# jonathan-laurent/AlphaZero.jl

Hardware: AMD Instinct MI355X
Metric: self-play MCTS sims/sec (Connect-Four, 4096 parallel games per GPU) (higher is better)
Workload: dtype f32

## Files before the change

alphazero.jl_amd/csrc/azhip.hip:

```cpp
#include "engine.h"

static thread_local std::string g_err;
int fail(int code, const char* fmt, ...) {
  char buf[512];
  va_list ap;
  va_start(ap, fmt);
  vsnprintf(buf, sizeof buf, fmt, ap);
  va_end(ap);
  g_err = buf;
  return code;
}
extern "C" const char* az_last_error(void) { return g_err.c_str(); }
extern "C" int az_abi_version(void) { return AZ_ABI_VERSION; }
extern "C" int az_abi_struct_size(int32_t which) {
  switch (which) {
    case AZ_STRUCT_ENGINE_CFG: return (int)sizeof(az_engine_cfg);
    case AZ_STRUCT_MOVE_REC: return (int)sizeof(az_move_rec);
    case AZ_STRUCT_GAME_REC: return (int)sizeof(az_game_rec);
    case AZ_STRUCT_TRACE_BUF: return (int)sizeof(az_trace_buf);
    case AZ_STRUCT_SELFPLAY_STATS: return (int)sizeof(az_selfplay_stats);
    case AZ_STRUCT_SAMPLE: return (int)sizeof(az_sample);
    case AZ_STRUCT_DATASET_INFO: return (int)sizeof(az_dataset_info);
    case AZ_STRUCT_LEARNING_STATUS: return (int)sizeof(az_learning_status_t);
    case AZ_STRUCT_TRAIN_CFG: return (int)sizeof(az_train_cfg);
// ... 48 lines not shown
  c->num_iters_per_turn = 600;
  c->temperature_len = 3;
  c->temperature_xs[0] = 0; c->temperature_xs[1] = 20; c->temperature_xs[2] = 30;
  c->temperature_ys[0] = 1.0; c->temperature_ys[1] = 1.0; c->temperature_ys[2] = 0.3;
  c->num_workers = 128; c->batch_size = 64; c->reset_every = 2; c->fill_batches = 1;
  c->flip_probability = 0.0; c->seed = 1;
  c->num_blocks = 5; c->num_filters = 64; c->num_policy_head_filters = 32; c->num_value_head_filters = 32;
  return AZ_OK;
}

static size_t net_nparams(const GameInfo& gi, const az_engine_cfg& c) {
  size_t P = gi.P, F = c.num_filters, npf = c.num_policy_head_filters, nvf = c.num_value_head_filters;
  size_t s = 9 * (size_t)gi.C * F + 5 * F;
  s += (size_t)c.num_blocks * 2 * (9 * F * F + 5 * F);
  s += F * npf + 5 * npf + (size_t)gi.A * P * npf + gi.A;
  s += F * nvf + 5 * nvf + F * P * nvf + F + F + 1;
  return s;
}

static void drop_wave_graphs(az_engine* e);
extern "C" int az_engine_destroy(az_engine* e) {
  if (!e) return AZ_OK;
  (void)hipSetDevice(e->device);
  if (e->ngroups == 1 && e->fr_s[0] && e->gs[0] == e->fr_s[0]) { for (int i = 0; i < 4; ++i) (void)hipStreamSynchronize(e->fr_s[i]); e->gs[0] = e->gt[0] = e->stream; }
  for (int g = 0; g < e->ngroups; ++g) if (e->gs[g] && e->gs[g] != e->stream) {
    (void)hipStreamSynchronize(e->gt[g]); (void)hipStreamSynchronize(e->gs[g]);
    (void)hipStreamDestroy(e->gt[g]); (void)hipStreamDestroy(e->gs[g]);
    (void)hipEventDestroy(e->ev_tree[g]); (void)hipEventDestroy(e->ev_net[g]);
  }
  if (e->stream) (void)hipStreamSynchronize(e->stream);
  split_register(e, 0);
  if (e->h_xflag) (void)hipHostFree(e->h_xflag);
  if (e->h_nleaf) (void)hipHostFree(e->h_nleaf);
  if (e->h_needy) (void)hipHostFree(e->h_needy);
  if (e->h_fr_words) (void)hipHostFree(e->h_fr_words);
  if (e->h_busy) (void)hipHostFree(e->h_busy);
  for (int i = 0; i < 4; ++i) { if (e->fr_s[i]) { (void)hipStreamSynchronize(e->fr_s[i]); (void)hipStreamDestroy(e->fr_s[i]); } if (e->fr_ev[i]) (void)hipEventDestroy(e->fr_ev[i]); }
  if (e->d_done) (void)hipFree(e->d_done);
  if (e->d_done_off) (void)hipFree(e->d_done_off);
  if (e->h_env) (void)hipHostFree(e->h_env);
  if (e->h_n) (void)hipHostFree(e->h_n);
  if (e->h_pv) (void)hipHostFree(e->h_pv);
  drop_wave_graphs(e);
  for (auto& r : e->prof_pool) { if (r.a) (void)hipEventDestroy(r.a); if (r.b) (void)hipEventDestroy(r.b); }
  for (void* q : e->net_allocs) (void)hipFree(q);
  for (void* q : e->allocs) (void)hipFree(q);
  if (e->d_phase) (void)hipFree(e->d_phase);
  for (size_t i = 0; i < e->vm_handles.size(); ++i) { (void)hipMemUnmap(e->vm_at[i], e->vm_chunk); (void)hipMemRelease(e->vm_handles[i]); }
  if (e->vm_base) (void)hipMemAddressFree(e->vm_base, e->vm_bytes);
  if (e->vmk_base) (void)hipMemAddressFree(e->vmk_base, e->vmk_bytes);
  if (e->stream) (void)hipStreamDestroy(e->stream);
  delete e;
  return AZ_OK;
}

__global__ void k_fill_u32(uint32_t* p, uint32_t val, int n) {
  int i = blockIdx.x * blockDim.x + threadIdx.x;
  if (i < n) p[i] = val;
}
__global__ void k_iota(int* p, int n) {
// ... 72 lines not shown
  if (c->temperature_len < 1 || c->temperature_len > AZ_SCHED_MAX) return fail(AZ_ERR_BAD_ARG, "temperature schedule needs 1..%d breakpoints", AZ_SCHED_MAX);
  if (c->reset_every < 0) return fail(AZ_ERR_BAD_ARG, "reset_every must be >= 0");
  if (c->lock_step != 0 && c->lock_step != 1) return fail(AZ_ERR_BAD_ARG, "lock_step must be 0 (free-running self-play) or 1");
  if (!(c->prior_temperature >= 0.0)) return fail(AZ_ERR_BAD_ARG, "prior_temperature must be >= 0");
  if (c->oracle == AZ_ORACLE_RESNET) {
    if (c->num_filters != 64 && c->num_filters != 128) return fail(AZ_ERR_BAD_ARG, "num_filters = %d: this build instantiates the 64- and 128-filter towers", c->num_filters);
    int hf = c->num_policy_head_filters + c->num_value_head_filters;
    if (c->num_policy_head_filters < 1 || c->num_value_head_filters < 1 || hf > c->num_filters) return fail(AZ_ERR_BAD_ARG, "head filters %d/%d unsupported (policy + value must be <= num_filters)", c->num_policy_head_filters, c->num_value_head_filters);
    if (c->num_blocks < 0 || c->num_blocks > 64) return fail(AZ_ERR_BAD_ARG, "num_blocks out of range");
    if (c->net_bf16 != 0 && c->net_bf16 != 1) return fail(AZ_ERR_BAD_ARG, "net_bf16 must be 0 or 1");
  }
  int ndev = 0;
  HIPCHK(hipGetDeviceCount(&ndev));
  if (c->device < 0 || c->device >= ndev) return fail(AZ_ERR_BAD_ARG, "device %d not available (%d visible)", c->device, ndev);
  HIPCHK(hipSetDevice(c->device));
  az_engine* e = new (std::nothrow) az_engine();
  if (!e) return fail(AZ_ERR_HIP, "out of host memory");
  e->cfg = *c; e->gi = gi; e->device = c->device; e->stream = nullptr; e->ngroups = 0; e->alloc_bytes = 0;
  e->vm_base = nullptr; e->vm_bytes = 0; e->vm_chunk = 0; e->vm_rows = 0; e->vm_chunk_nodes = 0; e->d_slot_cap = nullptr; e->vm_budget = 0; e->vm_mapped = 0;
  e->vmk_base = nullptr; e->vmk_bytes = 0; e->vmk_piece = 0; e->tree_sort = 0; e->d_perm = nullptr; e->d_perm_prev = nullptr;
  e->next_exec = 1.0;
  e->h_env = nullptr; e->h_n = nullptr; e->h_pv = nullptr; e->h_nleaf = nullptr; e->d_nleaf = nullptr; e->h_needy = nullptr; e->d_needy = nullptr;
  e->d_ec = nullptr; e->ec_mask = 0; e->ec_seq = 0; e->d_ec_claim = nullptr; e->d_Phit = nullptr; e->d_Vhit = nullptr;
  e->fr_on = false; e->fr_k = 0; e->fr_kbg = 0; e->fr_round_waves = 0; for (int i = 0; i < 4; ++i) { e->fr_s[i] = nullptr; e->fr_ev[i] = nullptr; } e->d_fr = nullptr; e->d_done = nullptr; e->d_done_off = nullptr; e->done_cap = 0;
  e->h_fr_words = nullptr; e->d_fr_words = nullptr; e->h_busy = nullptr; e->d_busy = nullptr; e->explore_k = 0; e->fr_prev_done = 0; e->fr_since_round = 0; e->fr_given_up = 0; e->fr_prev_recs = 0;
  e->h_xflag = nullptr; e->d_xflag = nullptr; e->split_off = false; e->split_registered = 0; e->xch_launches = 0;
  { const char* fa = getenv("AZHIP_XCH_FAIL_AT"); e->xch_fail_at = fa ? atoll(fa) : 0; }
  e->net_loaded = false; e->running = false; e->prof_on = false; { const char* ug = getenv("AZHIP_GRAPH"); e->use_graphs = ug ? atoi(ug) : 0; }
  e->d_phase = nullptr; e->phase_cap = 0; e->phase_n = 0; e->host_moves = true; e->last_tower[0] = 0; memset(e->tower_hist, 0, sizeof e->tower_hist); e->prof_mask = 0; e->prof_used = 0;
  memset(&e->prof, 0, sizeof e->prof);
  memset(&e->stats, 0, sizeof e->stats);
  int st = [&]() -> int {
    {
      int ncu = 0;
      HIPCHK(hipDeviceGetAttribute(&ncu, hipDeviceAttributeMultiprocessorCount, c->device));
      std::vector<uint32_t> mask((size_t)(ncu + 31) / 32, 0u);
      for (int i = 0; i < ncu; ++i) mask[(size_t)i / 32] |= 1u << (i % 32);
      if (getenv("AZHIP_POOLED_QUEUE") || ncu <= 0 || hipExtStreamCreateWithCUMask(&e->stream, (uint32_t)mask.size(), mask.data()) != hipSuccess) {
        (void)hipGetLastError();
        e->stream = nullptr;
        HIPCHK(hipStreamCreate(&e->stream));
      }
    }
    const int G = c->num_workers;
    DView& v = e->v;
    memset(&v, 0, sizeof v);
    v.G = G;
// ... 158 lines not shown
      gv.G = Gh; gv.slot0 = (int)o;
      gv.sr += o; gv.game_id += o; gv.move_idx += o;
      gv.worker_sim_id += o; gv.eta += o * gi.APAD;
      gv.ht += o * hs; gv.nodes += o * v.node_stride; gv.path += o * v.max_depth;
      if (gv.slot_cap) gv.slot_cap += o;
      gv.leaf_env += o; gv.eval_slots += o; gv.bg_list += o; gv.bg_cnt += 2 * g;
      if (gv.ec) { gv.ec_claim += 2 * o; gv.Phit += o * gi.APAD; gv.Vhit += o; }
      gv.xerr = e->d_xerr + g; gv.skipped = e->d_skipped + 2 * g;
      if (e->tree_sort) {
        gv.perm = e->d_perm + o;
        hipLaunchKernelGGL(k_iota, dim3((Gh + 255) / 256), dim3(256), 0, e->stream, e->d_perm + o, Gh);
      }
      gv.needy_host = e->d_needy + g;
      gv.nleaf_host = e->d_ec ? e->d_nleaf + g : nullptr;
      gv.n_eval += 2 * g; gv.keys += o * v.key_stride; gv.Pout += o * gi.APAD; gv.Vout += o; gv.trace += o * v.max_moves; gv.grec += o; gv.finished += o;
      e->gv[g] = gv;
      if (ng == 1) {
        e->gs[g] = e->gt[g] = e->stream;
        int lo = 0, hi = 0;
        HIPCHK(hipDeviceGetStreamPriorityRange(&lo, &hi));
        HIPCHK(hipStreamCreateWithPriority(&e->fr_s[0], hipStreamNonBlocking, hi));
        HIPCHK(hipStreamCreateWithPriority(&e->fr_s[1], hipStreamNonBlocking, hi));
        HIPCHK(hipStreamCreateWithPriority(&e->fr_s[2], hipStreamNonBlocking, hi));
        HIPCHK(hipStreamCreateWithPriority(&e->fr_s[3], hipStreamNonBlocking, hi));
        for (int i = 0; i < 4; ++i) HIPCHK(hipEventCreateWithFlags(&e->fr_ev[i], hipEventDisableTiming));
      } else {
        int lo = 0, hi = 0;
        HIPCHK(hipDeviceGetStreamPriorityRange(&lo, &hi));
        HIPCHK(hipStreamCreateWithPriority(&e->gs[g], hipStreamNonBlocking, hi));
        HIPCHK(hipStreamCreateWithPriority(&e->gt[g], hipStreamNonBlocking, lo));
        HIPCHK(hipEventCreateWithFlags(&e->ev_tree[g], hipEventDisableTiming));
        HIPCHK(hipEventCreateWithFlags(&e->ev_net[g], hipEventDisableTiming));
      }
      AZCHK(dalloc(e, &e->g_hfeat[g], (size_t)Gh * gi.P * std::max(64, c->num_filters), false));
      e->ngroups = g + 1;
    }
    DParams& p = e->p;
    memset(&p, 0, sizeof p);
    p.gamma = c->gamma; p.cpuct = c->cpuct; p.eps = c->dirichlet_noise_eps; p.alpha = c->dirichlet_noise_alpha;
    p.prior_temp = c->prior_temperature; p.nsims = c->num_iters_per_turn; p.temp_len = c->temperature_len;
    for (int i = 0; i < AZ_SCHED_MAX; ++i) { p.temp_xs[i] = c->temperature_xs[i]; p.temp_ys[i] = c->temperature_ys[i]; }
    p.seed = c->seed; p.oracle = c->oracle; p.reset_every = c->reset_every; p.retire = 0;
    p.flip_p = c->flip_probability;
    if (e->vm_rows) {
      size_t fr = 0, tot = 0;
      HIPCHK(hipMemGetInfo(&fr, &tot));
      const size_t margin = std::max<size_t>(tot / 8, (size_t)4 << 30);
      const char* gb = getenv("AZHIP_POOL_GB");
// ... 455 lines not shown
  if (side) { s2 = e->fr_s[1]; HIPCHK(hipEventRecord(e->fr_ev[0], st)); ++e->bg_seq; e->bg_signal = bg_stop_on && e->fr_kbg > 0; }
  if (e->cfg.oracle == AZ_ORACLE_RESNET) {
    AZCHK(net_wave(e, g, split, e->group_active[g]));
  } else {
    LAUNCH_ON(e, st, AZ_K_SYNTH, G, (k_synth_oracle<Gm>), (G + 255) / 256, 256, 0, v, e->p, sim_idx, par);
  }
  if (e->fr_on) {
    FRArgs fa;
    fa.st = e->d_fr; fa.done = e->d_done; fa.done_off = e->d_done_off;
    fa.recs = e->d_phase ? e->d_phase : e->d_stage; fa.recs_cap = e->d_phase ? (long long)e->phase_cap : (long long)e->v.G * e->v.max_moves;
    fa.done_cap = e->done_cap; fa.total_games = e->total_games; fa.first_game_id = (uint32_t)e->first_game_id; fa.group = g; fa.host_words = e->d_fr_words;
    static const int bg_prio = getenv("AZHIP_BG_PRIO") ? atoi(getenv("AZHIP_BG_PRIO")) : 0;
    hipStream_t s3 = side ? e->fr_s[2] : s2;
    if (side) { HIPCHK(hipStreamWaitEvent(s2, e->fr_ev[0], 0)); HIPCHK(hipStreamWaitEvent(s3, e->fr_ev[0], 0)); }
    { DView mv = v; mv.low_prio = bg_prio ? 0 : 1; LAUNCH_ON(e, s3, AZ_K_MOVE, G, (k_move_fr<Gm>), (G + 255) / 256, 256, 0, mv, e->p, fa); }
    if (e->fr_kbg > 0) {
      AZCHK(ec_next_launch(e, &e->gv[g]));
      DView bv = e->gv[g];
      bv.run_k = e->fr_kbg; bv.low_prio = bg_prio ? 0 : 1;
      if (side && e->bg_signal) { bv.bg_stop = e->d_bg_stop; bv.bg_seq = e->bg_seq; }
      LAUNCH_ON(e, s2, AZ_K_EXPAND, G, (k_tree<Gm>), gb, 256, 0, bv, e->p, 0, 1, par ^ 1);
    }
    if (side) {
      HIPCHK(hipEventRecord(e->fr_ev[1], s2)); HIPCHK(hipStreamWaitEvent(st, e->fr_ev[1], 0));
      HIPCHK(hipEventRecord(e->fr_ev[2], s3)); HIPCHK(hipStreamWaitEvent(st, e->fr_ev[2], 0));
    }
    else if (split && e->cfg.oracle == AZ_ORACLE_RESNET) HIPCHK(hipStreamWaitEvent(st, e->ev_net[g], 0));
  }
  return AZ_OK;
}
template <class Gm> static int recover_split(az_engine* e) {
  AZCHK(sync_all(e));
  *e->h_xflag = 0;
  int xerr[AZ_MAX_GROUPS + 1], skipped[2 * (AZ_MAX_GROUPS + 1)];
  HIPCHK(hipMemcpy(xerr, e->d_xerr, sizeof xerr, hipMemcpyDeviceToHost));
  HIPCHK(hipMemcpy(skipped, e->d_skipped, sizeof skipped, hipMemcpyDeviceToHost));
  HIPCHK(hipMemsetAsync(e->d_xerr, 0, sizeof xerr, e->stream));
  HIPCHK(hipMemsetAsync(e->d_skipped, 0, sizeof skipped, e->stream));
  HIPCHK(hipStreamSynchronize(e->stream));
  bool any = false;
  for (int g = 0; g < e->ngroups; ++g) any = any || xerr[g] == DERR_EXCHANGE;
  if (!any) return AZ_OK;
  e->split_off = true;
  e->stats.tower_fallbacks++;
  for (int g = 0; g < e->ngroups; ++g) {
    e->wave_par[g] ^= (skipped[2 * g] & 1);
    if (skipped[2 * g + 1]) e->pending[g] = true;
  }
// ... 589 lines not shown

extern "C" int az_selfplay_aborted(az_engine* e, int32_t* game_ids, int32_t cap, int32_t* n) {
  ENGINE(e);
  if (!n || (cap > 0 && !game_ids)) return fail(AZ_ERR_BAD_ARG, "NULL");
  *n = (int32_t)e->aborted_ids.size();
  if (*n > cap) return cap == 0 ? AZ_OK : fail(AZ_ERR_CAPACITY, "%d aborted games, room for %d", *n, cap);
  for (int i = 0; i < *n; ++i) game_ids[i] = e->aborted_ids[i];
  return AZ_OK;
}

extern "C" int az_selfplay_end(az_engine* e) {
  ENGINE(e);
  e->p.retire = 0;
  split_register(e, 0);
  if (!e->running) return AZ_OK;
  AZCHK(reset_wave_state(e));
  hipLaunchKernelGGL(k_slot_records, dim3((e->v.G + 255) / 256), dim3(256), 0, e->stream, e->v, (int)SR_CLEAR_ACTIVE);
  HIPCHK(hipStreamSynchronize(e->stream));
  e->running = false;
  e->active_slots = 0;
  e->fr_on = false;
  for (int g = 0; g < e->ngroups; ++g) { e->gv[g].run_k = 0; e->gv[g].fr = 0; e->gv[g].fr_active = nullptr; }
  if (e->ngroups == 1 && e->gs[0] != e->stream) {
    HIPCHK(hipStreamSynchronize(e->gs[0])); for (int i = 1; i < 4; ++i) HIPCHK(hipStreamSynchronize(e->fr_s[i]));
    e->gs[0] = e->gt[0] = e->stream;
  }
  return AZ_OK;
}

extern "C" int az_selfplay_run(az_engine* e, int32_t num_games, int32_t first_game_id, az_trace_buf* out,
                               az_progress_cb cb, void* user, az_selfplay_stats* stats) {
  ENGINE(e);
  if (num_games < 1 || !out) return fail(AZ_ERR_BAD_ARG, "num_games must be >= 1 and out non-NULL");
  if (out->games_cap < num_games) return fail(AZ_ERR_CAPACITY, "games_cap %lld < num_games %d", (long long)out->games_cap, num_games);
  e->host_moves = out->moves != nullptr;
  const int bst = az_selfplay_begin(e, num_games, first_game_id);
  if (bst != AZ_OK) { e->host_moves = true; return bst; }
  int reported = 0;
  int st = AZ_OK;
  while (e->games_done < num_games) {
    st = az_selfplay_step(e, e->fr_on ? e->fr_round_waves : e->p.nsims);
    if (st != AZ_OK) break;
    if (cb) for (; reported < e->games_done; ++reported) cb(user);
  }
  if (st == AZ_OK && stats) st = az_selfplay_get_stats(e, stats);
  std::string keep = g_err;
  const int cst = az_selfplay_collect(e, out);
// ... 257 lines not shown
```

alphazero.jl_amd/csrc/engine.h:

```cpp
#pragma once
#include <hip/hip_runtime.h>

#include <algorithm>
#include <chrono>
#include <cmath>
#include <cstdarg>
#include <cstdio>
#include <cstring>
#include <new>
#include <string>
#include <map>
#include <mutex>
#include <vector>
#include <unordered_set>

#include "../../include/az_numerics.h"
#include "../../include/azhip.h"
#include "games.h"
#include "resnet.h"
#include "resnet16.h"
#include "resnet16b.h"
#include "tree.h"

int fail(int code, const char* fmt, ...);
// ... 71 lines not shown
  int ntm;
  long long tower_hist[4];
  char last_tower[96];
  int heads_pick;
  int tower_pick;
  int num_cu;
  int nn_cap;
  float* d_hfeat; float* d_X; float* d_A; float* d_P; float* d_V; float* d_Pinv;
  GEnv* d_tmp_env; int* d_iota; int* d_ntmp;
  GEnv* h_env; int* h_n; float* h_pv;
  int* d_slots; uint32_t* d_gids; GEnv* d_roots; uint32_t* d_moves; double* d_eta; int* d_offsets;
  az_move_rec* d_stage; unsigned long long* d_keys; int* d_actions; unsigned long long* d_next; signed char* d_term; float* d_reward;
  char* d_nodebuf;
  int* d_visits;
  int io_cap;
  bool running;
  int total_games, next_game, first_game_id, games_done, wave_in_move, active_slots;
  std::map<int, hipGraphExec_t> wave_graphs; int use_graphs;
  bool pending[AZ_MAX_GROUPS];
  int wave_par[AZ_MAX_GROUPS];
  int group_active[AZ_MAX_GROUPS];
  bool fr_on;
  int fr_k, fr_kbg, fr_round_waves;
  hipStream_t fr_s[4]; hipEvent_t fr_ev[4];
  FRState* d_fr; az_game_rec* d_done; long long* d_done_off; int done_cap;
  int* h_busy; int* d_busy;
  int explore_k;
  int* d_bg_stop; int bg_seq; bool bg_signal;
  int* h_fr_words; int* d_fr_words;
  int fr_prev_done, fr_since_round, fr_given_up; long long fr_prev_recs;
  std::vector<az_game_rec> h_done; std::vector<long long> h_done_off;
  std::vector<az_game_rec> q_games;
  std::vector<az_move_rec> q_moves;
  az_move_rec* d_phase; int64_t phase_cap, phase_n; bool host_moves;
  std::vector<az_game_rec> ph_games;
  std::vector<int64_t> ph_off;
  az_selfplay_stats stats;
  std::chrono::steady_clock::time_point t_begin;
  bool prof_on;
  int prof_mask;
  std::vector<ProfRec> prof_pool;
  size_t prof_used;
  az_prof prof;
  double next_exec;
  std::vector<int> h_finished;
  std::vector<az_game_rec> h_grec;
};

template <class T> inline int dalloc(az_engine* e, T** p, size_t n, bool zero = true) {
  void* q = nullptr;
  size_t bytes = std::max<size_t>(n * sizeof(T), 16);
  hipError_t r = hipMalloc(&q, bytes);
  if (r != hipSuccess) return fail(AZ_ERR_HIP, "hipMalloc(%zu bytes) failed: %s", bytes, hipGetErrorString(r));
  e->allocs.push_back(q);
  e->alloc_bytes += bytes;
  if (zero) HIPCHK(hipMemsetAsync(q, 0, bytes, e->stream));
  *p = (T*)q;
  return AZ_OK;
}

inline int sync_groups(az_engine* e) {
  for (int g = 0; g < e->ngroups; ++g) if (e->gs[g] != e->stream) {
    HIPCHK(hipStreamSynchronize(e->gt[g]));
    HIPCHK(hipStreamSynchronize(e->gs[g]));
  }
  if (e->fr_on && e->fr_s[1]) for (int i = 1; i < 4; ++i) HIPCHK(hipStreamSynchronize(e->fr_s[i]));
  return AZ_OK;
}
inline int sync_all(az_engine* e) {
  AZCHK(sync_groups(e));
  HIPCHK(hipStreamSynchronize(e->stream));
  return AZ_OK;
}
inline int prof_flush(az_engine* e) {
  if (!e->prof_used) return AZ_OK;
  AZCHK(sync_all(e));
  for (size_t i = 0; i < e->prof_used; ++i) {
    float ms = 0.f;
    HIPCHK(hipEventElapsedTime(&ms, e->prof_pool[i].a, e->prof_pool[i].b));
    e->prof.ms[e->prof_pool[i].cls] += ms;
  }
  e->prof_used = 0;
  return AZ_OK;
}
inline int prof_begin(az_engine* e, hipStream_t st, int cls, int64_t units) {
  if (!e->prof_on || (e->prof_mask && !((e->prof_mask >> cls) & 1))) return AZ_OK;
  if (e->prof_used == e->prof_pool.size()) AZCHK(prof_flush(e));
  ProfRec& r = e->prof_pool[e->prof_used];
  r.cls = cls;
// ... 64 lines not shown
```

alphazero.jl_amd/csrc/net_impl.h:

```cpp
#pragma once
#include "engine.h"

template <class Gm, int F, bool PLANES_ONLY = false> static int set_kernel_attrs_f() {
  HIPCHK(hipFuncSetAttribute(reinterpret_cast<const void*>(&k_tower16<Gm, F, false>), hipFuncAttributeMaxDynamicSharedMemorySize, T16<Gm, F>::BYTES));
  HIPCHK(hipFuncSetAttribute(reinterpret_cast<const void*>(&k_tower16<Gm, F, true>), hipFuncAttributeMaxDynamicSharedMemorySize, T16<Gm, F>::BYTES));
  if constexpr (NTM<Gm> > 0) {
    HIPCHK(hipFuncSetAttribute(reinterpret_cast<const void*>(&k_tower16<Gm, F, false, NTM<Gm>>), hipFuncAttributeMaxDynamicSharedMemorySize, T16<Gm, F, NTM<Gm>>::BYTES));
    HIPCHK(hipFuncSetAttribute(reinterpret_cast<const void*>(&k_tower16<Gm, F, true, NTM<Gm>>), hipFuncAttributeMaxDynamicSharedMemorySize, T16<Gm, F, NTM<Gm>>::BYTES));
  }
  if constexpr (F == 64) {
    HIPCHK(hipFuncSetAttribute(reinterpret_cast<const void*>(&k_tower16x2<Gm, F, false>), hipFuncAttributeMaxDynamicSharedMemorySize, T16P<Gm, F>::BYTES));
    HIPCHK(hipFuncSetAttribute(reinterpret_cast<const void*>(&k_tower16x2<Gm, F, true>), hipFuncAttributeMaxDynamicSharedMemorySize, T16P<Gm, F>::BYTES));
    HIPCHK(hipFuncSetAttribute(reinterpret_cast<const void*>(&k_tower16x2<Gm, F, false, 10, 9>), hipFuncAttributeMaxDynamicSharedMemorySize, T16P<Gm, F, 10, 9>::BYTES));
    HIPCHK(hipFuncSetAttribute(reinterpret_cast<const void*>(&k_tower16x2<Gm, F, true, 10, 9>), hipFuncAttributeMaxDynamicSharedMemorySize, T16P<Gm, F, 10, 9>::BYTES));
    HIPCHK(hipFuncSetAttribute(reinterpret_cast<const void*>(&k_tower16x2m<Gm, F, false>), hipFuncAttributeMaxDynamicSharedMemorySize, T16P<Gm, F>::BYTES));
    HIPCHK(hipFuncSetAttribute(reinterpret_cast<const void*>(&k_tower16x2c<Gm, F, false>), hipFuncAttributeMaxDynamicSharedMemorySize, T16P<Gm, F>::BYTES));
    HIPCHK(hipFuncSetAttribute(reinterpret_cast<const void*>(&k_tower16x2c<Gm, F, true>), hipFuncAttributeMaxDynamicSharedMemorySize, T16P<Gm, F>::BYTES));
  }
  HIPCHK(hipFuncSetAttribute(reinterpret_cast<const void*>(&k_tower16b<Gm, F, false, 11>), hipFuncAttributeMaxDynamicSharedMemorySize, T16B<Gm, F, 11>::BYTES));
  HIPCHK(hipFuncSetAttribute(reinterpret_cast<const void*>(&k_tower16b<Gm, F, true, 11>), hipFuncAttributeMaxDynamicSharedMemorySize, T16B<Gm, F, 11>::BYTES));
  HIPCHK(hipFuncSetAttribute(reinterpret_cast<const void*>(&k_tower16b<Gm, F, false, NTS<Gm>>), hipFuncAttributeMaxDynamicSharedMemorySize, T16B<Gm, F, NTS<Gm>>::BYTES));
  HIPCHK(hipFuncSetAttribute(reinterpret_cast<const void*>(&k_tower16b<Gm, F, true, NTS<Gm>>), hipFuncAttributeMaxDynamicSharedMemorySize, T16B<Gm, F, NTS<Gm>>::BYTES));
  if constexpr (F == 128) {
    HIPCHK(hipFuncSetAttribute(reinterpret_cast<const void*>(&k_tower16b<Gm, F, false, 22>), hipFuncAttributeMaxDynamicSharedMemorySize, T16B<Gm, F, 22>::BYTES));
// ... 263 lines not shown
        e->next_exec = (first * tower_exec_frac<Gm, F>(e, 21) + (seen - first) * tower_exec_frac<Gm, F>(e, 19)) / (double)seen;
        LAUNCH_ON(e, sn, AZ_K_TOWER, N, (k_tower16x2m<Gm, F, false>), cu + (N - first + T19::TB - 1) / T19::TB, THR21, LDS21, e->net16, v.leaf_env, eslots, nev, N, (const float*)nullptr, e->g_hfeat[g], cu);
        snprintf(e->last_tower, sizeof e->last_tower, "k_tower16x2m<%s,%d>", Gm::ID == 0 ? "ConnectFour" : Gm::ID == 1 ? "TicTacToe" : "Mancala", F);
      } else if (rounds_on && e->tower_pick == 0 && N > first && seen > first && seen + 16 <= first + cu * T19::TB) {
        LAUNCH_ON(e, sn, AZ_K_TOWER, first, (k_tower16x2<Gm, F, false>), cu, THR21, LDS21, e->net16, v.leaf_env, eslots, nev, N, (const float*)nullptr, e->g_hfeat[g], 0);
        e->next_exec = tower_exec_frac<Gm, F>(e, 19);
        LAUNCH_ON(e, sn, AZ_K_TOWER, N - first, (k_tower16x2<Gm, F, false, 10, 9>), (N - first + T19::TB - 1) / T19::TB, (T19::THREADS), (T19::BYTES), e->net16, v.leaf_env, eslots, nev, N, (const float*)nullptr, e->g_hfeat[g], first);
      } else {
        LAUNCH_ON(e, sn, AZ_K_TOWER, N, (k_tower16x2<Gm, F, false>), (N + TB21 - 1) / TB21, THR21, LDS21, e->net16, v.leaf_env, eslots, nev, N, (const float*)nullptr, e->g_hfeat[g], 0);
      }
    }
  } else if (tw == 7) {
    if constexpr (NTM<Gm> > 0) {
      using TM = T16<Gm, F, NTM<Gm>>;
      LAUNCH_ON(e, sn, AZ_K_TOWER, N, (k_tower16<Gm, F, false, NTM<Gm>>), (N + TM::TB - 1) / TM::TB, THR16, (TM::BYTES), e->net16, v.leaf_env, eslots, nev, N, (const float*)nullptr, e->g_hfeat[g]);
    }
  } else if (tw == 3)
    LAUNCH_ON(e, sn, AZ_K_TOWER, N, (k_tower16<Gm, F, false, NTS<Gm>>), (N + TB3 - 1) / TB3, THR16, LDS3, e->net16, v.leaf_env, eslots, nev, N, (const float*)nullptr, e->g_hfeat[g]);
  else if (tw == 16)
    LAUNCH_ON(e, sn, AZ_K_TOWER, N, (k_tower16<Gm, F, false>), (N + TB16 - 1) / TB16, THR16, LDS16, e->net16, v.leaf_env, eslots, nev, N, (const float*)nullptr, e->g_hfeat[g]);
  else
    LAUNCH_ON(e, sn, AZ_K_TOWER, N, (k_tower<Gm, F, false>), (N + TB - 1) / TB, TowerCfg<F>::THREADS, TowerLds<F>::BYTES, e->net, v.leaf_env, eslots, nev, N, (const float*)nullptr, e->g_hfeat[g]);
  const bool fr = e->fr_on && split;
  if (e->bg_signal) {
    HIPCHK(hipEventRecord(e->fr_ev[3], sn));
    HIPCHK(hipStreamWaitEvent(e->fr_s[3], e->fr_ev[3], 0));
    hipLaunchKernelGGL(k_set_word, dim3(1), dim3(1), 0, e->fr_s[3], e->d_bg_stop, e->bg_seq);
  }
  if (split && !fr) { HIPCHK(hipEventRecord(e->ev_net[g], sn)); HIPCHK(hipStreamWaitEvent(st, e->ev_net[g], 0)); }
  AZCHK((launch_heads<Gm, F>(e, fr ? sn : st, e->g_hfeat[g], v.leaf_env, eslots, nev, N, (const float*)nullptr, v.Pout, v.Vout, (float*)nullptr, L)));
  if (fr) HIPCHK(hipEventRecord(e->ev_net[g], sn));
  return AZ_OK;
}
template <class Gm> static int wave_net(az_engine* e, int g, bool split, int nmax) {
  return e->cfg.num_filters == 128 ? wave_net_f<Gm, 128>(e, g, split, nmax) : wave_net_f<Gm, 64>(e, g, split, nmax);
}

#define AZ_NET_GAME_TU(Gm, sfx)                                                                                              \
  int net_set_kernel_attrs_##sfx(az_engine* e) { return set_kernel_attrs<Gm>(e); }                                                      \
  int net_launch_##sfx(az_engine* e, hipStream_t st, bool from_planes, float* hfeat, const GEnv* envs, const int* eslots,    \
                       const int* n_ptr, int n_max, const float* X, const float* Amask, float* Pout, float* Vout, float* Pinv, \
                       int pstride) {                                                                                        \
    return from_planes ? launch_net<Gm, true>(e, st, hfeat, envs, eslots, n_ptr, n_max, X, Amask, Pout, Vout, Pinv, pstride)  \
                       : launch_net<Gm, false>(e, st, hfeat, envs, eslots, n_ptr, n_max, X, Amask, Pout, Vout, Pinv, pstride); \
  }                                                                                                                          \
  int net_wave_##sfx(az_engine* e, int g, bool split, int nmax) { return wave_net<Gm>(e, g, split, nmax); }                  \
  int net_geometry_##sfx(int which, uint16_t* out, int64_t cap, int* rows, int* products) {                                  \
    return which == 0 ? geometry_out<typename T16<Gm, 64, 11>::Geo>(out, cap, rows, products)                                \
         : which == 1 ? geometry_out<typename T16<Gm, 64, NTS<Gm>>::Geo>(out, cap, rows, products)                                 \
         : which == 2 ? geometry_out<typename T16P<Gm, 64>::Geo>(out, cap, rows, products)                                   \
                      : geometry_out<typename T16B<Gm, 128, 22>::Geo>(out, cap, rows, products);                             \
  }
```

alphazero.jl_amd/csrc/resnet.h:

```cpp
#pragma once
#include <hip/hip_runtime.h>
#include <stdint.h>
#include "../../include/az_numerics.h"
#include "games.h"

typedef float f32x16 __attribute__((ext_vector_type(16)));
typedef float f32x4v __attribute__((ext_vector_type(4)));

template <int I, int N, class Fn> __device__ __forceinline__ void static_for_impl(Fn& f) {
  if constexpr (I < N) { f(std::integral_constant<int, I>{}); static_for_impl<I + 1, N>(f); }
}
template <int N, class Fn> __device__ __forceinline__ void static_for(Fn f) { static_for_impl<0, N>(f); }

struct NetDev {
  int nblocks, F, npf, nvf, HF;
  const float* stem_w;
  const float* stem_ss;
  const float4* conv_w;
  const float* conv_ss;
  const float4* head_w;
  const float* head_ss;
  const float* pol_w;
  const float* pol_b;
  const float* val_w;
  const float* val_b;
  const float* val2_w;
  float val2_b;
  unsigned long long* dbg;
  const float2* hd_w;
  int hd_ok;
  const float4* hd16_w;
  int hd16_ok;
};

static constexpr int TOWER_ROWS = 128;

template <int F> struct TowerLds {
  static constexpr int STRIDE = F + 4;
  static constexpr int BUF = (TOWER_ROWS + 1) * STRIDE;
  static constexpr int BYTES = 2 * BUF * 4;
};

template <int F>
__device__ __forceinline__ void load_b_tap(const float4* __restrict__ wt, float4 (&b)[F / 8]) {
#pragma unroll
  for (int jq = 0; jq < F / 8; ++jq) b[jq] = wt[(size_t)jq * 64];
}
template <int F>
__device__ __forceinline__ void mfma_tap(const float4 (&af)[2], const float* __restrict__ arow0,
                                         const float* __restrict__ arow1, const float4 (&b)[F / 8], f32x16 (&acc)[2]) {
#pragma unroll
  for (int c0 = 0; c0 < F / 8; c0 += 8) {
    float4 a0[8], a1[8];
#pragma unroll
    for (int jq = 0; jq < 8; ++jq) {
      if (c0 == 0 && jq == 0) { a0[0] = af[0]; a1[0] = af[1]; }
// ... 249 lines not shown
  av = av + net.val2_b;
  Vout[e] = az_tanhf(av);
}
template <class Gm, int F>
__device__ __forceinline__ void heads_finish(const NetDev& net, const GEnv* __restrict__ leaf_env, const int* __restrict__ eval_slots,
                                             const float* __restrict__ Amask, float* __restrict__ Pout, float* __restrict__ Vout,
                                             float* __restrict__ Pinv, int pstride, int e, const float* __restrict__ logit, const float* __restrict__ vh) {
  heads_finish_policy<Gm>(leaf_env, eval_slots, Amask, Pout, Pinv, pstride, e, logit);
  heads_finish_value<F>(net, Vout, e, vh);
}

template <class Gm> constexpr int HEADS_LP = (Gm::A + 15) / 16 * 16;
template <class Gm> constexpr int HEADS_NPT = (Gm::A + 31) / 32;
template <class Gm, int F>
__global__ void __launch_bounds__(4 * (F + HEADS_LP<Gm>))
k_heads(NetDev net, const GEnv* __restrict__ leaf_env, const int* __restrict__ eval_slots,
        const int* __restrict__ n_eval_ptr, int n_fixed, const float* __restrict__ Amask,
        const float* __restrict__ hfeat, float* __restrict__ Pout, float* __restrict__ Vout,
        float* __restrict__ Pinv, int pstride) {
  constexpr int P = Gm::P, A = Gm::A, HB = 4, PER = F + HEADS_LP<Gm>;
  static_assert(F + A <= PER, "thread map");
  __shared__ float s_logit[HB][HEADS_LP<Gm>];
  __shared__ float s_vh[HB][F];
  const int n = n_eval_ptr ? *n_eval_ptr : n_fixed;
  const int board0 = blockIdx.x * HB;
  if (board0 >= n) return;
  const int b = threadIdx.x / PER, o = threadIdx.x % PER;
  const int e = board0 + b;
  const int HF = net.HF;
  if (e < n && o < F + A) {
    const float* hf = hfeat + (size_t)e * P * HF;
    float acc = 0.0f;
    if (o < F) {
      const int nvf = net.nvf;
      const float* w = net.val_w + o;
      for (int q = 0; q < P; ++q) {
        const float* h = hf + q * HF + net.npf;
        for (int f = 0; f < nvf; ++f) acc = az_fmaf(h[f], w[(size_t)(q * nvf + f) * F], acc);
      }
      acc = acc + net.val_b[o];
      s_vh[b][o] = acc > 0.0f ? acc : 0.0f;
    } else {
      const int a = o - F, npf = net.npf;
      const float* w = net.pol_w + a;
      for (int q = 0; q < P; ++q) {
        const float* h = hf + q * HF;
// ... 67 lines not shown
  for (int r = 0; r < 16; ++r) {
    const int row = (r & 3) + 8 * (r >> 2) + 4 * h;
    if (is_pol) { if (pt * 32 + col < A) s_logit[row * LP + pt * 32 + col] = acc[r] + net.pol_b[pt * 32 + col]; }
    else {
      const int o = wave * 32 + col;
      const float v = acc[r] + net.val_b[o];
      s_vh[row * SV + o] = v > 0.0f ? v : 0.0f;
    }
  }
  }
  __syncthreads();
  const int b = threadIdx.x;
  if (b < 32 && board0 + b < n) heads_finish<Gm, F>(net, leaf_env, eval_slots, Amask, Pout, Vout, Pinv, pstride, board0 + b, s_logit + b * LP, s_vh + b * SV);
}
template <class Gm, int F>
__global__ void __launch_bounds__(64 * (F / 32 + HEADS_NPT<Gm>))
k_heads_mfma(NetDev net, const GEnv* __restrict__ leaf_env, const int* __restrict__ eval_slots,
             const int* __restrict__ n_eval_ptr, int n_fixed, const float* __restrict__ Amask,
             const float* __restrict__ hfeat, float* __restrict__ Pout, float* __restrict__ Vout,
             float* __restrict__ Pinv, int pstride) {
  __builtin_amdgcn_s_setprio(3);
  __shared__ float s_vh[32 * (F + 1)];
  __shared__ float s_logit[32 * HEADS_LP<Gm>];
  const int n = n_eval_ptr ? *n_eval_ptr : n_fixed;
  const int board0 = blockIdx.x * 32;
  if (board0 >= n) return;
  heads_mfma_tile<Gm, F>(net, leaf_env, eval_slots, n, Amask, hfeat, Pout, Vout, Pinv, pstride, board0, s_vh, s_logit);
}

#ifndef HEADS16_DEPTH
#define HEADS16_DEPTH 8
#endif
#ifndef HEADS16_WDEPTH
#define HEADS16_WDEPTH 16
#endif
template <class Gm> constexpr int HEADS16_NPT = (Gm::A + 15) / 16;
template <class Gm, int F, bool SPLIT> struct H16 {
  static constexpr int P = Gm::P, NVT = F / 16, NPT = HEADS16_NPT<Gm>;
  static constexpr int WAVES = SPLIT ? (NVT > NPT ? NVT : NPT) : NVT + NPT, THREADS = 64 * WAVES;
  static constexpr int NB = 2 * P, RS = 20, SV = F + 1, LP = HEADS_LP<Gm>;
  static constexpr bool STAGE = SPLIT && 16 * P * 32 * 4 <= 96 * 1024;
  static constexpr int A_FLOATS = STAGE ? NB * 256 : 0, PATCH_FLOATS = STAGE ? 0 : WAVES * 3 * 16 * RS;
  static constexpr int BYTES = (A_FLOATS + PATCH_FLOATS + 16 * SV + 16 * LP) * 4;
};
template <class Gm, int F, bool SPLIT> struct H16Threads { static constexpr int V = H16<Gm, F, SPLIT>::THREADS; };
template <class Gm, int F, bool SPLIT>
__global__ void __launch_bounds__((H16Threads<Gm, F, SPLIT>::V))
k_heads16(NetDev net, const GEnv* __restrict__ leaf_env, const int* __restrict__ eval_slots,
          const int* __restrict__ n_eval_ptr, int n_fixed, const float* __restrict__ Amask,
          const float* __restrict__ hfeat, float* __restrict__ Pout, float* __restrict__ Vout,
          float* __restrict__ Pinv, int pstride) {
  using H = H16<Gm, F, SPLIT>;
  constexpr int P = Gm::P, A = Gm::A, NVT = H::NVT, NPT = H::NPT, LP = H::LP, SV = H::SV, NB = H::NB, RS = H::RS;
  __builtin_amdgcn_s_setprio(3);
  extern __shared__ __attribute__((aligned(16))) float h16_lds[];
  float* As = h16_lds;
  float* s_tr = h16_lds + H::A_FLOATS;
  float* s_vh = s_tr + H::PATCH_FLOATS;
  float* s_logit = s_vh + 16 * SV;
  const int n = n_eval_ptr ? *n_eval_ptr : n_fixed;
  const int board0 = (SPLIT ? (int)blockIdx.x >> 1 : (int)blockIdx.x) * 16;
  if (board0 >= n) return;
  const int lane = threadIdx.x & 63, wave = threadIdx.x >> 6, m = lane & 15, g = lane >> 4;
  unsigned long long* dbg = (net.dbg && lane == 0) ? net.dbg + ((size_t)blockIdx.x * H::WAVES + wave) * 4 : nullptr;
  if (dbg) dbg[0] = __builtin_readcyclecounter();
  const bool is_pol = SPLIT ? (blockIdx.x & 1) != 0 : wave < NPT;
  const int pt = wave, vt = SPLIT ? wave : wave - NPT;
  const bool active = !SPLIT || wave < (is_pol ? NPT : NVT);
  const int HF = net.HF, foff = is_pol ? 0 : net.npf;
  if constexpr (H::STAGE) {
    for (int idx = threadIdx.x; idx < 16 * P * 8; idx += H::THREADS) {
      const int c = idx & 7, p = (idx >> 3) % P, b = idx / (8 * P);
      int eb = board0 + b;
      if (eb >= n) eb = n - 1;
      const f32x4v v = *(const f32x4v*)(hfeat + ((size_t)eb * P + p) * HF + foff + 4 * c);
      float* dst = As + ((2 * p + (c >> 2)) * 16 + b) * 16 + (c & 3);
      const int rot = 2 * ((b >> 2) & 1);
      dst[4 * ((0 + rot) & 3)] = v.x; dst[4 * ((1 + rot) & 3)] = v.y; dst[4 * ((2 + rot) & 3)] = v.z; dst[4 * ((3 + rot) & 3)] = v.w;
    }
    __syncthreads();
  }
  if (active) {
// ... 109 lines not shown
```

alphazero.jl_amd/csrc/tree.h:

```cpp
#pragma once
#include <hip/hip_runtime.h>
#include <stdint.h>
#include <type_traits>
#include "../../include/az_numerics.h"
#include "../../include/azhip.h"
#include "games.h"

enum { LEAF_NONE = 0, LEAF_NEW = 1, LEAF_TERMINAL = 2 };
enum { DERR_NODE_POOL = 1, DERR_HASH_FULL = 2, DERR_DEPTH = 3, DERR_MOVES = 4, DERR_NO_ROOT = 5 };

struct DParams {
  double gamma, cpuct, eps, alpha, prior_temp;
  int nsims, temp_len;
  int temp_xs[AZ_SCHED_MAX];
  double temp_ys[AZ_SCHED_MAX];
  uint64_t seed;
  int oracle, reset_every;
  double flip_p;
  int retire;
};

enum { SR_ACTIVE = 1, SR_MS_SHIFT = 8 };
struct alignas(64) SlotRec {
  unsigned long long root_a, root_b;
// ... 232 lines not shown
  typename NL::hi_t* hp = (typename NL::hi_t*)(nd + NL::OFF_HI);
  *hp = (typename NL::hi_t)((*hp & ~((typename NL::hi_t)3 << (2 * act))) | ((typename NL::hi_t)(link >> 16) << (2 * act)));
}

struct KArgs { DView v; DParams p; };
template <class Gm>
__global__ void __launch_bounds__(256) __attribute__((amdgpu_num_vgpr(160))) k_tree(DView v_arg, DParams p_arg, int do_backup, int do_select, int par) {
  if (!v_arg.low_prio) __builtin_amdgcn_s_setprio(3);
  const DView& v = v_arg;
  constexpr int L = Gm::APAD;
  using NL = NodeL<Gm>;
  __shared__ int s_new[4], s_hit[4], s_evl[4], s_sims[4], s_trav[4], s_need[4], s_base, s_nbase;
  const int tid = blockIdx.x * blockDim.x + threadIdx.x;
  const int lgrp = tid / L, lane = tid % L;
  const int wl = threadIdx.x & 63, w = threadIdx.x >> 6, gbase = wl & ~(L - 1);
  int nlive = v.G;
  const int* map = v.perm;
  if (v.fr && !do_backup && v.bg_list) { nlive = v.bg_cnt[par ^ 1]; map = v.bg_list + (size_t)(par ^ 1) * v.eval_stride; }
  const bool live = lgrp < nlive;
  const int slot_in = live ? (map ? map[lgrp] : lgrp) : 0;
  const bool links_ok = v.cap_nodes <= LINK_MAX;
  unsigned long long* dbg = (v.dbg && blockIdx.x == 0 && threadIdx.x == 0) ? v.dbg : nullptr;
  if (dbg) dbg[0] = __builtin_readcyclecounter();
  if (__hip_atomic_load(v.xerr, __ATOMIC_RELAXED, __HIP_MEMORY_SCOPE_AGENT) == (int)DERR_EXCHANGE) {
    if (blockIdx.x == 0 && threadIdx.x == 0 && (do_backup || !v.fr)) atomicAdd(v.skipped + (do_select ? 0 : 1), 1);
    return;
  }

  const SlotRec s0 = v.sr[slot_in];
  unsigned long long st = (v.path + (size_t)slot_in * v.max_depth)[lane < v.max_depth ? lane : 0];
  GEnv lenv = v.leaf_env[slot_in];
  int kind = s0.leaf_kd & 3, depth = (s0.leaf_kd >> 2) & 0x0fffffff, e0 = s0.eidx, nc = s0.node_count;
  GEnv root0 = s0.root();
  uint32_t epoch0 = s0.epoch, ins = s0.leaf_ins;
  int ridx = s0.root_idx, active0 = s0.active;
  int claim0 = -1; uint32_t cmeta0 = 0;
  if (v.ec) { const int2 c2 = ((const int2*)v.ec_claim)[slot_in]; claim0 = c2.x; cmeta0 = (uint32_t)c2.y; }
#define AZ_PIN(x) asm volatile("" : "+v"(x))
  AZ_PIN(kind); AZ_PIN(depth); AZ_PIN(e0); AZ_PIN(nc); AZ_PIN(st); AZ_PIN(root0.a); AZ_PIN(root0.b); AZ_PIN(root0.fin);
  AZ_PIN(epoch0); AZ_PIN(ins); AZ_PIN(claim0); AZ_PIN(cmeta0); AZ_PIN(lenv.a); AZ_PIN(lenv.b); AZ_PIN(lenv.fin); AZ_PIN(ridx); AZ_PIN(active0);
  const bool mine = live && !(v.fr && kind != LEAF_NONE && (!do_backup || ((s0.leaf_kd >> 30) & 1) == par));
  if (!(do_backup && mine)) kind = LEAF_NONE;
  const int nc_in = nc, ridx_in = ridx;
  const bool inrec = lane < Gm::A;
  float Pans = 0.f, Vans = 0.f;
  if (kind == LEAF_NEW) {
    Pans = e0 >= 0 ? v.Pout[(size_t)e0 * L + lane] : v.Phit[(size_t)slot_in * L + lane];
// ... 606 lines not shown
  const int slot = slots[i];
  uint32_t ep = v.sr[slot].epoch + 1;
  if (ep >= 0xffff) {
    unsigned long long* tab = v.ht + (size_t)slot * v.ht_size;
    for (int k = 0; k < v.ht_size; ++k) tab[k] = 0;
    ep = 1;
  }
  v.sr[slot].epoch = ep;
  v.sr[slot].node_count = 0;
  v.sr[slot].root_idx = -1;
}

enum { SR_CLEAR_ACTIVE = 1, SR_CLEAR_LEAF = 2, SR_CLEAR_TOTALS = 4, SR_RESET_TREE = 8, SR_ZERO = 16 };
static __global__ void __launch_bounds__(256) k_slot_records(DView v, int what) {
  const int slot = blockIdx.x * blockDim.x + threadIdx.x;
  if (slot >= v.G) return;
  SlotRec* const sr = v.sr + slot;
  if (what & SR_ZERO) { SlotRec z = {}; z.epoch = v.epoch0; z.root_idx = -1; *sr = z; return; }
  if (what & SR_CLEAR_ACTIVE) sr->active = 0;
  if (what & SR_CLEAR_LEAF) sr->leaf_kd = LEAF_NONE;
  if (what & SR_CLEAR_TOTALS) { sr->tot_sims = 0; sr->tot_trav = 0; }
  if (what & SR_RESET_TREE) { sr->node_count = 0; sr->epoch = v.epoch0; sr->root_idx = -1; }
}
static __global__ void k_set_word(int* p, int val) { __hip_atomic_store(p, val, __ATOMIC_RELAXED, __HIP_MEMORY_SCOPE_AGENT); }
static __global__ void __launch_bounds__(256) k_node_counts(DView v, int* out) {
  const int slot = blockIdx.x * blockDim.x + threadIdx.x;
  if (slot < v.G) out[slot] = v.sr[slot].node_count;
}

static __global__ void __launch_bounds__(1024) k_depth_order(DView v, long long* prev , int* perm , int* kbuf ) {
  __shared__ int bins[64], base[64];
  const int t = threadIdx.x;
  if (t < 64) bins[t] = 0;
  __syncthreads();
  for (int s = t; s < v.G; s += blockDim.x) {
    const SlotRec* r = v.sr + s;
    const long long tt = r->tot_trav, ts = r->tot_sims;
    const long long dt = tt - prev[2 * s], ds = ts - prev[2 * s + 1];
    prev[2 * s] = tt; prev[2 * s + 1] = ts;
    int k = 63;
    if (r->active) { const long long h = ds > 0 ? 2 * dt / ds : 0; k = h < 0 ? 0 : h > 62 ? 62 : (int)h; }
    kbuf[s] = k;
    atomicAdd(&bins[k], 1);
  }
  __syncthreads();
  if (t == 0) { int acc = 0; for (int k = 0; k < 64; ++k) { base[k] = acc; acc += bins[k]; } }
  __syncthreads();
// ... 35 lines not shown
```

Baseline: 8.834 million.

## Fold background-stop signal into heads kernel and drop fourth stream

Removes the dedicated fourth stream and its one-thread k_set_word launch that signalled the background tree work to stop. The heads kernels now store the stop word themselves when a stop pointer is passed. The side-stream join is rechained so s3 feeds s2 before s2 feeds the main stream, and the xerr check in the non-backup tree kernel is read once per block through shared memory. The stop signal now fires when the heads kernel starts rather than right after the tower, which changes overlap timing, and the added __syncthreads sits on a per-block path.

```diff
diff --git a/alphazero.jl_amd/csrc/azhip.hip b/alphazero.jl_amd/csrc/azhip.hip
--- a/alphazero.jl_amd/csrc/azhip.hip
+++ b/alphazero.jl_amd/csrc/azhip.hip
@@ -94,7 +94,7 @@
 extern "C" int az_engine_destroy(az_engine* e) {
   if (!e) return AZ_OK;
   (void)hipSetDevice(e->device);
-  if (e->ngroups == 1 && e->fr_s[0] && e->gs[0] == e->fr_s[0]) { for (int i = 0; i < 4; ++i) (void)hipStreamSynchronize(e->fr_s[i]); e->gs[0] = e->gt[0] = e->stream; }
+  if (e->ngroups == 1 && e->fr_s[0] && e->gs[0] == e->fr_s[0]) { for (int i = 0; i < 3; ++i) (void)hipStreamSynchronize(e->fr_s[i]); e->gs[0] = e->gt[0] = e->stream; }
   for (int g = 0; g < e->ngroups; ++g) if (e->gs[g] && e->gs[g] != e->stream) {
     (void)hipStreamSynchronize(e->gt[g]); (void)hipStreamSynchronize(e->gs[g]);
     (void)hipStreamDestroy(e->gt[g]); (void)hipStreamDestroy(e->gs[g]);
@@ -107,7 +107,7 @@
   if (e->h_needy) (void)hipHostFree(e->h_needy);
   if (e->h_fr_words) (void)hipHostFree(e->h_fr_words);
   if (e->h_busy) (void)hipHostFree(e->h_busy);
-  for (int i = 0; i < 4; ++i) { if (e->fr_s[i]) { (void)hipStreamSynchronize(e->fr_s[i]); (void)hipStreamDestroy(e->fr_s[i]); } if (e->fr_ev[i]) (void)hipEventDestroy(e->fr_ev[i]); }
+  for (int i = 0; i < 3; ++i) { if (e->fr_s[i]) { (void)hipStreamSynchronize(e->fr_s[i]); (void)hipStreamDestroy(e->fr_s[i]); } if (e->fr_ev[i]) (void)hipEventDestroy(e->fr_ev[i]); }
   if (e->d_done) (void)hipFree(e->d_done);
   if (e->d_done_off) (void)hipFree(e->d_done_off);
   if (e->h_env) (void)hipHostFree(e->h_env);
@@ -226,7 +226,7 @@
   e->next_exec = 1.0;
   e->h_env = nullptr; e->h_n = nullptr; e->h_pv = nullptr; e->h_nleaf = nullptr; e->d_nleaf = nullptr; e->h_needy = nullptr; e->d_needy = nullptr;
   e->d_ec = nullptr; e->ec_mask = 0; e->ec_seq = 0; e->d_ec_claim = nullptr; e->d_Phit = nullptr; e->d_Vhit = nullptr;
-  e->fr_on = false; e->fr_k = 0; e->fr_kbg = 0; e->fr_round_waves = 0; for (int i = 0; i < 4; ++i) { e->fr_s[i] = nullptr; e->fr_ev[i] = nullptr; } e->d_fr = nullptr; e->d_done = nullptr; e->d_done_off = nullptr; e->done_cap = 0;
+  e->fr_on = false; e->fr_k = 0; e->fr_kbg = 0; e->fr_round_waves = 0; for (int i = 0; i < 3; ++i) { e->fr_s[i] = nullptr; e->fr_ev[i] = nullptr; } e->d_fr = nullptr; e->d_done = nullptr; e->d_done_off = nullptr; e->done_cap = 0;
   e->h_fr_words = nullptr; e->d_fr_words = nullptr; e->h_busy = nullptr; e->d_busy = nullptr; e->explore_k = 0; e->fr_prev_done = 0; e->fr_since_round = 0; e->fr_given_up = 0; e->fr_prev_recs = 0;
   e->h_xflag = nullptr; e->d_xflag = nullptr; e->split_off = false; e->split_registered = 0; e->xch_launches = 0;
   { const char* fa = getenv("AZHIP_XCH_FAIL_AT"); e->xch_fail_at = fa ? atoll(fa) : 0; }
@@ -431,8 +431,7 @@
         HIPCHK(hipStreamCreateWithPriority(&e->fr_s[0], hipStreamNonBlocking, hi));
         HIPCHK(hipStreamCreateWithPriority(&e->fr_s[1], hipStreamNonBlocking, hi));
         HIPCHK(hipStreamCreateWithPriority(&e->fr_s[2], hipStreamNonBlocking, hi));
-        HIPCHK(hipStreamCreateWithPriority(&e->fr_s[3], hipStreamNonBlocking, hi));
-        for (int i = 0; i < 4; ++i) HIPCHK(hipEventCreateWithFlags(&e->fr_ev[i], hipEventDisableTiming));
+        for (int i = 0; i < 3; ++i) HIPCHK(hipEventCreateWithFlags(&e->fr_ev[i], hipEventDisableTiming | hipEventReleaseToDevice));
       } else {
         int lo = 0, hi = 0;
         HIPCHK(hipDeviceGetStreamPriorityRange(&lo, &hi));
@@ -934,8 +933,8 @@
       LAUNCH_ON(e, s2, AZ_K_EXPAND, G, (k_tree<Gm>), gb, 256, 0, bv, e->p, 0, 1, par ^ 1);
     }
     if (side) {
+      HIPCHK(hipEventRecord(e->fr_ev[2], s3)); HIPCHK(hipStreamWaitEvent(s2, e->fr_ev[2], 0));
       HIPCHK(hipEventRecord(e->fr_ev[1], s2)); HIPCHK(hipStreamWaitEvent(st, e->fr_ev[1], 0));
-      HIPCHK(hipEventRecord(e->fr_ev[2], s3)); HIPCHK(hipStreamWaitEvent(st, e->fr_ev[2], 0));
     }
     else if (split && e->cfg.oracle == AZ_ORACLE_RESNET) HIPCHK(hipStreamWaitEvent(st, e->ev_net[g], 0));
   }
@@ -1571,7 +1570,7 @@
   e->fr_on = false;
   for (int g = 0; g < e->ngroups; ++g) { e->gv[g].run_k = 0; e->gv[g].fr = 0; e->gv[g].fr_active = nullptr; }
   if (e->ngroups == 1 && e->gs[0] != e->stream) {
-    HIPCHK(hipStreamSynchronize(e->gs[0])); for (int i = 1; i < 4; ++i) HIPCHK(hipStreamSynchronize(e->fr_s[i]));
+    HIPCHK(hipStreamSynchronize(e->gs[0])); for (int i = 1; i < 3; ++i) HIPCHK(hipStreamSynchronize(e->fr_s[i]));
     e->gs[0] = e->gt[0] = e->stream;
   }
   return AZ_OK;
diff --git a/alphazero.jl_amd/csrc/engine.h b/alphazero.jl_amd/csrc/engine.h
--- a/alphazero.jl_amd/csrc/engine.h
+++ b/alphazero.jl_amd/csrc/engine.h
@@ -117,7 +117,7 @@
   int group_active[AZ_MAX_GROUPS];
   bool fr_on;
   int fr_k, fr_kbg, fr_round_waves;
-  hipStream_t fr_s[4]; hipEvent_t fr_ev[4];
+  hipStream_t fr_s[3]; hipEvent_t fr_ev[3];
   FRState* d_fr; az_game_rec* d_done; long long* d_done_off; int done_cap;
   int* h_busy; int* d_busy;
   int explore_k;
@@ -159,7 +159,7 @@
     HIPCHK(hipStreamSynchronize(e->gt[g]));
     HIPCHK(hipStreamSynchronize(e->gs[g]));
   }
-  if (e->fr_on && e->fr_s[1]) for (int i = 1; i < 4; ++i) HIPCHK(hipStreamSynchronize(e->fr_s[i]));
+  if (e->fr_on && e->fr_s[1]) for (int i = 1; i < 3; ++i) HIPCHK(hipStreamSynchronize(e->fr_s[i]));
   return AZ_OK;
 }
 inline int sync_all(az_engine* e) {
diff --git a/alphazero.jl_amd/csrc/net_impl.h b/alphazero.jl_amd/csrc/net_impl.h
--- a/alphazero.jl_amd/csrc/net_impl.h
+++ b/alphazero.jl_amd/csrc/net_impl.h
@@ -309,13 +309,11 @@
   else
     LAUNCH_ON(e, sn, AZ_K_TOWER, N, (k_tower<Gm, F, false>), (N + TB - 1) / TB, TowerCfg<F>::THREADS, TowerLds<F>::BYTES, e->net, v.leaf_env, eslots, nev, N, (const float*)nullptr, e->g_hfeat[g]);
   const bool fr = e->fr_on && split;
-  if (e->bg_signal) {
-    HIPCHK(hipEventRecord(e->fr_ev[3], sn));
-    HIPCHK(hipStreamWaitEvent(e->fr_s[3], e->fr_ev[3], 0));
-    hipLaunchKernelGGL(k_set_word, dim3(1), dim3(1), 0, e->fr_s[3], e->d_bg_stop, e->bg_seq);
-  }
+  if (e->bg_signal) { e->net.bg_stop = e->d_bg_stop; e->net.bg_seq = e->bg_seq; }
   if (split && !fr) { HIPCHK(hipEventRecord(e->ev_net[g], sn)); HIPCHK(hipStreamWaitEvent(st, e->ev_net[g], 0)); }
-  AZCHK((launch_heads<Gm, F>(e, fr ? sn : st, e->g_hfeat[g], v.leaf_env, eslots, nev, N, (const float*)nullptr, v.Pout, v.Vout, (float*)nullptr, L)));
+  const int hrc = launch_heads<Gm, F>(e, fr ? sn : st, e->g_hfeat[g], v.leaf_env, eslots, nev, N, (const float*)nullptr, v.Pout, v.Vout, (float*)nullptr, L);
+  e->net.bg_stop = nullptr;
+  AZCHK(hrc);
   if (fr) HIPCHK(hipEventRecord(e->ev_net[g], sn));
   return AZ_OK;
 }
diff --git a/alphazero.jl_amd/csrc/resnet.h b/alphazero.jl_amd/csrc/resnet.h
--- a/alphazero.jl_amd/csrc/resnet.h
+++ b/alphazero.jl_amd/csrc/resnet.h
@@ -31,7 +31,11 @@
   int hd_ok;
   const float4* hd16_w;
   int hd16_ok;
+  int* bg_stop; int bg_seq;
 };
+__device__ __forceinline__ void heads_stop_background(const NetDev& net) {
+  if (net.bg_stop && blockIdx.x == 0 && threadIdx.x == 0) __hip_atomic_store(net.bg_stop, net.bg_seq, __ATOMIC_RELAXED, __HIP_MEMORY_SCOPE_AGENT);
+}
 
 static constexpr int TOWER_ROWS = 128;
 
@@ -327,6 +331,7 @@
   static_assert(F + A <= PER, "thread map");
   __shared__ float s_logit[HB][HEADS_LP<Gm>];
   __shared__ float s_vh[HB][F];
+  heads_stop_background(net);
   const int n = n_eval_ptr ? *n_eval_ptr : n_fixed;
   const int board0 = blockIdx.x * HB;
   if (board0 >= n) return;
@@ -440,6 +445,7 @@
   __builtin_amdgcn_s_setprio(3);
   __shared__ float s_vh[32 * (F + 1)];
   __shared__ float s_logit[32 * HEADS_LP<Gm>];
+  heads_stop_background(net);
   const int n = n_eval_ptr ? *n_eval_ptr : n_fixed;
   const int board0 = blockIdx.x * 32;
   if (board0 >= n) return;
@@ -476,6 +482,7 @@
   float* s_tr = h16_lds + H::A_FLOATS;
   float* s_vh = s_tr + H::PATCH_FLOATS;
   float* s_logit = s_vh + 16 * SV;
+  heads_stop_background(net);
   const int n = n_eval_ptr ? *n_eval_ptr : n_fixed;
   const int board0 = (SPLIT ? (int)blockIdx.x >> 1 : (int)blockIdx.x) * 16;
   if (board0 >= n) return;
diff --git a/alphazero.jl_amd/csrc/tree.h b/alphazero.jl_amd/csrc/tree.h
--- a/alphazero.jl_amd/csrc/tree.h
+++ b/alphazero.jl_amd/csrc/tree.h
@@ -278,7 +278,16 @@
   const bool links_ok = v.cap_nodes <= LINK_MAX;
   unsigned long long* dbg = (v.dbg && blockIdx.x == 0 && threadIdx.x == 0) ? v.dbg : nullptr;
   if (dbg) dbg[0] = __builtin_readcyclecounter();
-  if (__hip_atomic_load(v.xerr, __ATOMIC_RELAXED, __HIP_MEMORY_SCOPE_AGENT) == (int)DERR_EXCHANGE) {
+  bool xgone;
+  if (v.fr && !do_backup) {
+    __shared__ int s_xerr;
+    if (threadIdx.x == 0) s_xerr = __hip_atomic_load(v.xerr, __ATOMIC_RELAXED, __HIP_MEMORY_SCOPE_AGENT);
+    __syncthreads();
+    xgone = s_xerr == (int)DERR_EXCHANGE;
+  } else {
+    xgone = __hip_atomic_load(v.xerr, __ATOMIC_RELAXED, __HIP_MEMORY_SCOPE_AGENT) == (int)DERR_EXCHANGE;
+  }
+  if (xgone) {
     if (blockIdx.x == 0 && threadIdx.x == 0 && (do_backup || !v.fr)) atomicAdd(v.skipped + (do_select ? 0 : 1), 1);
     return;
   }
@@ -931,7 +940,6 @@
   if (what & SR_CLEAR_TOTALS) { sr->tot_sims = 0; sr->tot_trav = 0; }
   if (what & SR_RESET_TREE) { sr->node_count = 0; sr->epoch = v.epoch0; sr->root_idx = -1; }
 }
-static __global__ void k_set_word(int* p, int val) { __hip_atomic_store(p, val, __ATOMIC_RELAXED, __HIP_MEMORY_SCOPE_AGENT); }
 static __global__ void __launch_bounds__(256) k_node_counts(DView v, int* out) {
   const int slot = blockIdx.x * blockDim.x + threadIdx.x;
   if (slot < v.G) out[slot] = v.sr[slot].node_count;
```

Result: faster. 8.971 million, median of 6 (+1.5%).
